# ziqin-h/GIVEPose

Measured on AMD Instinct MI355X. Metric: images/sec PoseNet fwd, bs=64 256x256 fp16, 1/2/4/8 MI355X; % MFMA roofline, higher is better.
Workload: dtype f16

## Files before the change

givepose_amd/_lib.py:

```python
import ctypes
import os
from ctypes import POINTER, Structure, c_char_p, c_double, c_float, c_int, c_long, c_void_p

_HERE = os.path.dirname(os.path.abspath(__file__))
LIB_PATH = os.environ.get("GP_LIB_PATH") or os.path.join(_HERE, "libgivepose_hip.so")

ABI_VERSION = 328
GP_F32, GP_F16, GP_F64 = 0, 1, 2
ACT_NONE, ACT_GELU, ACT_RELU, ACT_LRELU = 0, 1, 2, 3
EPI_NONE, EPI_GELU, EPI_RELU, EPI_LRELU, EPI_SCALE_RES, EPI_RES_RELU, EPI_LNFOLD_GELU = 0, 1, 2, 3, 4, 5, 6
ROT_6D, ROT_6D_Y, ROT_6D_Z, ROT_QUAT, ROT_EULER = 0, 1, 2, 3, 4
KC_GEMM, KC_DCNV3, KC_DWCONV_LN, KC_NORM, KC_ELEMENTWISE, KC_SMALL, KC_COUNT = 0, 1, 2, 3, 4, 5, 6
KC_NAMES = ["gemm", "dcnv3", "dwconv_ln", "norm", "elementwise", "small"]


class GemmDesc(Structure):
    _fields_ = [("X", c_void_p), ("W", c_void_p), ("bias", c_void_p), ("gamma", c_void_p), ("residual", c_void_p),
                ("C", c_void_p), ("workspace", c_void_p),
                ("M", c_int), ("N", c_int), ("K", c_int), ("ldx", c_int), ("ldc", c_int), ("ldres", c_int),
                ("epilogue", c_int), ("out_f32", c_int), ("splitk", c_int),
                ("B", c_int), ("H", c_int), ("Win", c_int), ("Cin", c_int), ("KH", c_int), ("KW", c_int),
                ("stride", c_int), ("pad", c_int), ("Ho", c_int), ("Wo", c_int), ("dtype", c_int),
                ("gn_partial", c_void_p), ("gn_groups", c_int), ("gn_hw", c_int), ("variant", c_int),
                ("ln_stats", c_void_p), ("ln_colsum", c_void_p), ("ln_nslab", c_int), ("ln_eps", c_float),
# ... 339 lines not shown
}
GPR_CHUNK, GPR_REPACK_LAUNCHES, GPR_REPACK_LAUNCHES_F32, GPR_MAX_ENTRIES, GPR_MAX_DIMS = 4096, 4, 3, 65536, 4
GPR_KIND_F32, GPR_KIND_F16, GPR_KIND_SPLIT = 0, 1, 2

TRAINDATA_PROTOTYPES = {
    "gpt_crop_train": ([_P] * 21 + [c_int] * 7 + [_P], c_int),
    "gpt_mask_deform": ([_P] * 3 + [c_ulonglong, _P, c_int, c_int, _P], c_int),
}
GPT_MAX_PIXELS, GPT_TRAIN_BATCH_LAUNCHES = 65536, 2

WPACK_PROTOTYPES = {
    "gpw_conv3_pack_wcm": ([_P, _P, c_int, c_int, _P], c_int),
    "gpw_gemm_desc_bytes": ([], c_int),
}

COLORAUG_PROTOTYPES = {
    "gpca_luma_partials": ([_P] * 5 + [c_int] * 3 + [_P], c_int),
    "gpca_apply": ([_P] * 6 + [c_int] * 3 + [_P], c_int),
}
GPCA_OP_SKIP, GPCA_OP_NONE, GPCA_OP_SHARPNESS, GPCA_OP_CONTRAST, GPCA_OP_BRIGHTNESS, GPCA_OP_COLOR = -1, 0, 1, 2, 3, 4
GPCA_BUF_FRAMES, GPCA_BUF_TMP0, GPCA_BUF_TMP1, GPCA_BUF_OUT = 0, 1, 2, 3
GPCA_PARTIALS, GPCA_STAGE_LAUNCHES, GPCA_MAX_FRAMES = 64, 2, 65535

_lib = None


class GivePoseHipError(RuntimeError):
    pass


# ... 2 lines not shown
    if _lib is not None:
        return _lib
    if not os.path.exists(LIB_PATH):
        raise GivePoseHipError(
            f"{LIB_PATH} not found: build it with `python -m givepose_amd.build` (hipcc --offload-arch=gfx950). "
            "There is no CPU or PyTorch fallback for the product path.")
    lib = ctypes.CDLL(LIB_PATH)
    for name, (argtypes, restype) in (list(PROTOTYPES.items()) + list(ALIGN_PROTOTYPES.items()) + list(LOSS_PROTOTYPES.items())
                                      + list(GRAD_PROTOTYPES.items()) + list(HEADGRAD_PROTOTYPES.items())
                                      + list(XYZGRAD_PROTOTYPES.items()) + list(XYZGRAD_BF16_PROTOTYPES.items()) + list(ENCGRAD_PROTOTYPES.items())
                                      + list(ENCGRAD_ORDERED_PROTOTYPES.items())
                                      + list(BBGRAD_PROTOTYPES.items()) + list(BBGRAD_BF16_PROTOTYPES.items()) + list(OPTIM_PROTOTYPES.items())
                                      + list(SIZEGRAD_PROTOTYPES.items()) + list(ACCUM_PROTOTYPES.items())
                                      + list(REPACK_PROTOTYPES.items()) + list(TRAINDATA_PROTOTYPES.items())
                                      + list(ADAM_PROTOTYPES.items()) + list(WPACK_PROTOTYPES.items())
                                      + list(COLORAUG_PROTOTYPES.items())):
        fn = getattr(lib, name)
        fn.argtypes = argtypes
        fn.restype = restype
    if lib.gp_version() != ABI_VERSION:
        raise GivePoseHipError(f"{LIB_PATH}: ABI version {lib.gp_version()}, this package needs {ABI_VERSION}: rebuild with "
                               "`python -m givepose_amd.build`")
    if lib.gpw_gemm_desc_bytes() != ctypes.sizeof(GemmDesc):
        raise GivePoseHipError(f"{LIB_PATH}: gp_gemm_desc is {lib.gpw_gemm_desc_bytes()} bytes there, {ctypes.sizeof(GemmDesc)} here: rebuild with "
                               "`python -m givepose_amd.build`")
    _lib = lib
    return lib


def check(rc, what=""):
    if rc != 0:
# ... 10 lines not shown
```

givepose_amd/build.py:

```python
import os
import subprocess
import sys

HERE = os.path.dirname(os.path.abspath(__file__))
CSRC = os.path.join(HERE, "csrc")
OBJ = os.path.join(HERE, "csrc", "build")
LIB = os.path.join(HERE, "libgivepose_hip.so")
SOURCES = ["runtime.hip", "gemm.hip", "mlp.hip", "dcnv3.hip", "dcnv3_any.hip", "norm.hip", "misc.hip", "scalenet.hip", "evalmap.hip", "align.hip", "loss.hip", "lossgrad.hip", "pnpgrad.hip", "xyzgrad.hip", "encgrad.hip", "encscatter.hip", "bbgrad.hip", "optim.hip", "sizegrad.hip", "accum.hip", "repack.hip", "traindata.hip", "adam.hip", "coloraug.hip"]
HIPCC = os.environ.get("HIPCC", "/opt/rocm/bin/hipcc")
FLAGS = ["-O3", "--offload-arch=gfx950", "-fPIC", "-std=c++17", "-Wno-unused-value"]
if os.environ.get("GP_PACKED_FP32") != "1":
    FLAGS += ["-Xclang", "-target-feature", "-Xclang", "-packed-fp32-ops", "-Wno-unknown-warning-option"]
EXTRA = os.environ.get("GP_EXTRA_HIPCC_FLAGS", "").split()
TAG = os.environ.get("GP_BUILD_TAG", "")
if EXTRA and not TAG:
    raise RuntimeError("GP_EXTRA_HIPCC_FLAGS needs GP_BUILD_TAG: an investigation build must not overwrite the product library")
if TAG:
    OBJ = os.path.join(HERE, "csrc", "build", "tag_" + TAG)
    LIB = os.path.join(HERE, f"libgivepose_hip_{TAG}.so")
    FLAGS += EXTRA


def _newer(a, b):
    return not os.path.exists(b) or os.path.getmtime(a) > os.path.getmtime(b)
# ... 1 lines not shown

def build(force=False, verbose=True):
    os.makedirs(OBJ, exist_ok=True)
    deps = [os.path.join(CSRC, "common.hpp"), os.path.join(HERE, "..", "include", "givepose_hip.h"),
            os.path.join(HERE, "..", "include", "givepose_align.h"), os.path.join(CSRC, "align_math.hpp"),
            os.path.join(HERE, "..", "include", "givepose_loss.h"), os.path.join(HERE, "..", "include", "givepose_grad.h"),
            os.path.join(HERE, "..", "include", "givepose_headgrad.h"), os.path.join(HERE, "..", "include", "givepose_xyzgrad.h"),
            os.path.join(HERE, "..", "include", "givepose_encgrad.h"), os.path.join(HERE, "..", "include", "givepose_bbgrad.h"),
            os.path.join(HERE, "..", "include", "givepose_optim.h"), os.path.join(HERE, "..", "include", "givepose_sizegrad.h"),
            os.path.join(HERE, "..", "include", "givepose_accum.h"), os.path.join(HERE, "..", "include", "givepose_repack.h"),
            os.path.join(HERE, "..", "include", "givepose_traindata.h"), os.path.join(CSRC, "grad_gemm.hpp"), os.path.join(CSRC, "grad_gemm_bf16.hpp"),
            os.path.join(HERE, "..", "include", "givepose_bbgrad_bf16.h"), os.path.join(CSRC, "xyz_conv_prec.hpp"),
            os.path.join(HERE, "..", "include", "givepose_xyzgrad_bf16.h"),
            os.path.join(HERE, "..", "include", "givepose_encgrad_ordered.h"), os.path.join(CSRC, "encscatter.hpp"),
            os.path.join(HERE, "..", "include", "givepose_adam.h"), os.path.join(HERE, "..", "include", "givepose_wpack.h"),
            os.path.join(HERE, "..", "include", "givepose_coloraug.h")]
    objs, procs = [], []
    for src in SOURCES:
        s, o = os.path.join(CSRC, src), os.path.join(OBJ, src.replace(".hip", ".o"))
        objs.append(o)
        if force or _newer(s, o) or any(_newer(d, o) for d in deps):
            if verbose:
                print("hipcc", src, flush=True)
            procs.append((src, subprocess.Popen([HIPCC, *FLAGS, "-c", s, "-o", o])))
    for src, p in procs:
        if p.wait() != 0:
            raise RuntimeError(f"hipcc failed on {src}")
    if force or procs or not os.path.exists(LIB) or any(_newer(o, LIB) for o in objs):
        subprocess.check_call([HIPCC, "--offload-arch=gfx950", "-shared", "-fPIC", "-o", LIB, *objs])
        if verbose:
            print("linked", LIB)
# ... 6 lines not shown
```

givepose_amd/csrc/mlp.hip:

```cpp
#include "common.hpp"

namespace {

struct MlpKP {
    const half_t* X;
    const half_t* W1;
    const float* b1;
    const half_t* W2p;
    const float* b2;
    const float* gamma;
    const half_t* res;
    half_t* out;
    int M;
    int dbg;
};

typedef __attribute__((address_space(3))) char lds_char_t;

__device__ __forceinline__ void glds16(const void* gsrc, unsigned lds_addr) {
    unsigned keep;
    asm volatile("s_mov_b32 %0, m0\n\ts_mov_b32 m0, %2\n\ts_nop 0\n\tglobal_load_lds_dwordx4 %1, off\n\ts_mov_b32 m0, %0"
                 : "=&s"(keep)
                 : "v"(gsrc), "s"(lds_addr)
                 : "memory");
}

__device__ __forceinline__ void glds16_sb(const void* sbase, unsigned voff, unsigned lds_addr) {
    unsigned keep;
    asm volatile("s_mov_b32 %0, m0\n\ts_mov_b32 m0, %3\n\ts_nop 0\n\tglobal_load_lds_dwordx4 %1, %2\n\ts_mov_b32 m0, %0"
// ... 8 lines not shown

#ifndef GP_MLP_WGS
#define GP_MLP_WGS 3
#endif
template <int C, int G16, int NWV = 8>
__global__ __launch_bounds__(NWV * 64, NWV == 4 ? GP_MLP_WGS : 1) void convnext_mlp_kernel(const MlpKP p) {
    constexpr int HD = 4 * C, NCH = HD / 32, KS = C / 32, CT = C / 16, MT = 2;
    constexpr int ROWB = C * 2;
    constexpr int W1B = 32 * ROWB, W2B = C * 64;
    constexpr int STAGE = W1B + W2B, NS = (NWV == 4 && C == 256) ? 2 : (NWV == 4 && GP_MLP_WGS == 3) ? 3 : 4, LEAD = NS - 1;
    constexpr int I1 = W1B / 1024 / NWV, I2 = W2B / 1024 / NWV, G = I1 + I2;
    constexpr int CPR1 = ROWB / 16, RPI1 = 64 / CPR1;
    constexpr int PITCH = ROWB + 16, SLAB = 32 * PITCH;
    constexpr int RING = NS * STAGE, SMEM = (RING + HD * 4) > NWV * SLAB ? (RING + HD * 4) : NWV * SLAB;
    static_assert(SMEM <= 160 * 1024, "LDS");
    __shared__ __attribute__((aligned(1024))) char smem[SMEM];

    const int tid = threadIdx.x, lane = tid & 63;
    const int wave = __builtin_amdgcn_readfirstlane(tid >> 6);
    const int fr = lane & 15, fq = lane >> 4;
    const long m0 = (long)xcd_chunk(blockIdx.x, gridDim.x) * (NWV * 32) + wave * 32;

    float* b1s = reinterpret_cast<float*>(smem + RING);
    for (int i = tid; i < HD / 4; i += NWV * 64) reinterpret_cast<f32x4*>(b1s)[i] = reinterpret_cast<const f32x4*>(p.b1)[i];

    uint4 xf[MT][KS];
#pragma unroll
    for (int mt = 0; mt < MT; ++mt)
#pragma unroll
        for (int ks = 0; ks < KS; ++ks)
            xf[mt][ks] = *reinterpret_cast<const uint4*>(p.X + (m0 + mt * 16 + fr) * C + ks * 32 + fq * 8);

    constexpr bool SB = true;
    unsigned w1off[I1], w2off[I2];
#pragma unroll
    for (int i = 0; i < I1; ++i) {
        const int r = (i * NWV + wave) * RPI1 + lane / CPR1, pc = lane % CPR1;
        w1off[i] = (unsigned)((r * C + ((pc ^ (r & 15)) << 3)) * 2);
    }
#pragma unroll
    for (int i = 0; i < I2; ++i) {
        const int lr = lane >> 2, r = (i * NWV + wave) * 16 + lr;
        w2off[i] = (unsigned)((r * HD + (((lane & 3) ^ ((-(lr >> 2)) & 3)) << 3)) * 2);
    }
    const unsigned lds0 = (unsigned)(size_t)(lds_char_t*)smem;
    auto stage = [&](int buf, int ch) {
        const unsigned s1 = lds0 + buf * STAGE + wave * 1024, s2 = s1 + W1B;
        const char* b1p = reinterpret_cast<const char*>(p.W1) + (long)ch * W1B;
        const char* b2p = reinterpret_cast<const char*>(p.W2p) + (long)ch * 64;
#pragma unroll
        for (int i = 0; i < I1; ++i) {
            if constexpr (SB) glds16_sb(b1p, w1off[i], s1 + i * NWV * 1024);
            else glds16(b1p + w1off[i], s1 + i * NWV * 1024);
        }
#pragma unroll
        for (int i = 0; i < I2; ++i) {
            if constexpr (SB) glds16_sb(b2p, w2off[i], s2 + i * NWV * 1024);
            else glds16(b2p + w2off[i], s2 + i * NWV * 1024);
        }
    };

    f32x4 acc2[CT][MT];
#pragma unroll
    for (int ct = 0; ct < CT; ++ct) {
        const f32x4 b = *reinterpret_cast<const f32x4*>(p.b2 + ct * 16 + fq * 4);
#pragma unroll
        for (int mt = 0; mt < MT; ++mt) acc2[ct][mt] = b;
    }
    __syncthreads();

#pragma unroll
    for (int i = 0; i < LEAD; ++i) stage(i, i);

    const int w1fo = fr * ROWB, w2fo = fr * 64 + ((fq ^ ((-(fr >> 2)) & 3)) << 4);
    int buf = 0, nbuf = LEAD;
    for (int ch = 0; ch < NCH; ++ch) {
        if (LEAD >= 3 && ch + 2 < NCH) asm volatile("s_waitcnt vmcnt(%0)" ::"n"(2 * G) : "memory");
        else if (LEAD >= 2 && ch + 1 < NCH) asm volatile("s_waitcnt vmcnt(%0)" ::"n"(G) : "memory");
        else asm volatile("s_waitcnt vmcnt(0)" ::: "memory");
        __builtin_amdgcn_s_barrier();
        __builtin_amdgcn_sched_barrier(0);
        if (ch + LEAD < NCH && p.dbg != 2) stage(nbuf, ch + LEAD);
        const char* s1 = smem + buf * STAGE + w1fo;
        const char* s2 = smem + buf * STAGE + W1B + w2fo;

        constexpr int GK = KS > 4 ? 1 : KS;
        f32x4 acc1[2][MT];
#pragma unroll
        for (int nt = 0; nt < 2; ++nt) {
            const f32x4 b = *reinterpret_cast<const f32x4*>(b1s + ch * 32 + nt * 16 + fq * 4);
#pragma unroll
            for (int mt = 0; mt < MT; ++mt) acc1[nt][mt] = b;
        }
#pragma unroll
        for (int k0 = 0; k0 < KS; k0 += GK) {
            uint4 a1[GK][2];
#pragma unroll
            for (int ks = 0; ks < GK; ++ks)
#pragma unroll
                for (int nt = 0; nt < 2; ++nt)
                    a1[ks][nt] = *reinterpret_cast<const uint4*>(s1 + nt * 16 * ROWB + ((((k0 + ks) * 4 + fq) ^ fr) << 4));
            __builtin_amdgcn_sched_barrier(0);
#pragma unroll
            for (int ks = 0; ks < GK; ++ks)
#pragma unroll
                for (int nt = 0; nt < 2; ++nt)
#pragma unroll
                    for (int mt = 0; mt < MT; ++mt) acc1[nt][mt] = mma16(a1[ks][nt], xf[mt][k0 + ks], acc1[nt][mt]);
            __builtin_amdgcn_sched_barrier(0);
        }
        constexpr int GC = CT > 8 ? 2 : (NWV == 4 && GP_MLP_WGS == 3) ? 4 : CT;
        uint4 a2[GC];
#pragma unroll
        for (int ct = 0; ct < GC; ++ct) a2[ct] = *reinterpret_cast<const uint4*>(s2 + ct * 1024);
        __builtin_amdgcn_sched_barrier(0);
        f32x2 v[8];
#pragma unroll
        for (int mt = 0; mt < MT; ++mt)
#pragma unroll
            for (int nt = 0; nt < 2; ++nt) {
                v[(mt * 2 + nt) * 2 + 0] = f32x2{acc1[nt][mt][0], acc1[nt][mt][1]};
                v[(mt * 2 + nt) * 2 + 1] = f32x2{acc1[nt][mt][2], acc1[nt][mt][3]};
            }
        uint4 hb[MT];
// ... 37 lines not shown
#pragma unroll
        for (int c0 = 0; c0 < CT; c0 += GC) {
            if (c0 > 0) {
#pragma unroll
                for (int ct = 0; ct < GC; ++ct) a2[ct] = *reinterpret_cast<const uint4*>(s2 + (c0 + ct) * 1024);
                __builtin_amdgcn_sched_barrier(0);
            }
#pragma unroll
            for (int ct = 0; ct < GC; ++ct)
#pragma unroll
                for (int mt = 0; mt < MT; ++mt) acc2[c0 + ct][mt] = mma16(a2[ct], hb[mt], acc2[c0 + ct][mt]);
            __builtin_amdgcn_sched_barrier(0);
        }
        buf = buf + 1 == NS ? 0 : buf + 1;
        nbuf = nbuf + 1 == NS ? 0 : nbuf + 1;
    }
    __syncthreads();

    constexpr int LPR = ROWB / 16, RPS = 64 / LPR, NIT = 32 / RPS;
    const int rr = lane / LPR, rc = lane % LPR;
    half8 rres[NIT];
    if constexpr (C == 128) {
#pragma unroll
        for (int i = 0; i < NIT; ++i) rres[i] = *reinterpret_cast<const half8*>(p.res + (m0 + i * RPS + rr) * C + rc * 8);
    }
    char* slab = smem + wave * SLAB;
#pragma unroll
    for (int ct = 0; ct < CT; ++ct) {
        const f32x4 g = *reinterpret_cast<const f32x4*>(p.gamma + ct * 16 + fq * 4);
#pragma unroll
// ... 415 lines not shown
    if (e != hipSuccess) return gp_fail(GP_ERR_LAUNCH, "gp_convnext_mlp_pack_w2_s32: %s", hipGetErrorString(e));
    return GP_OK;
}

extern "C" int gp_convnext_mlp_pack_w2(const void* w2, void* w2p, int C, void* stream) {
    GP_REQUIRE(w2 && w2p && w2 != w2p, "gp_convnext_mlp_pack_w2: bad pointers");
    GP_REQUIRE(C == 128 || C == 256 || C == 512, "gp_convnext_mlp_pack_w2: C=%d must be 128, 256 or 512", C);
    const long n = (long)C * 4 * C;
    hipLaunchKernelGGL(mlp_pack_w2_kernel, dim3(cdiv(n, 256)), dim3(256), 0, (hipStream_t)stream,
                       reinterpret_cast<const half_t*>(w2), reinterpret_cast<half_t*>(w2p), C, 4 * C);
    hipError_t e = hipGetLastError();
    if (e != hipSuccess) return gp_fail(GP_ERR_LAUNCH, "gp_convnext_mlp_pack_w2: %s", hipGetErrorString(e));
    return GP_OK;
}

extern "C" int gp_convnext_mlp(const void* x, const void* w1, const float* b1, const void* w2p, const float* b2,
                               const float* gamma, const void* residual, void* out, long M, int C, int dtype_in, void* stream) {
    const bool s32 = (dtype_in & GP_MLP_S32) != 0;
    const int dtype = dtype_in & ~GP_MLP_S32;
    GP_REQUIRE(dtype == GP_F16, "gp_convnext_mlp: fp16 storage only (fp32 runs fc1 / fc2 through gp_gemm)");
    GP_REQUIRE(!s32 || (C == 128 && gp_gelu16_enabled()), "gp_convnext_mlp: GP_MLP_S32 exists for C = 128 with the packed-fp16 GELU");
    GP_REQUIRE(C == 128 || C == 256 || C == 512, "gp_convnext_mlp: C=%d must be 128, 256 or 512", C);
    GP_REQUIRE(M > 0 && M % (C == 512 ? 128 : 256) == 0, "gp_convnext_mlp: M=%ld must be a positive multiple of %d", M, C == 512 ? 128 : 256);
    GP_REQUIRE(x && w1 && b1 && w2p && b2 && gamma && residual && out, "gp_convnext_mlp: null operand");
    GP_REQUIRE((((size_t)x | (size_t)w1 | (size_t)w2p | (size_t)residual | (size_t)out | (size_t)b1 | (size_t)b2 | (size_t)gamma) & 15) == 0,
               "gp_convnext_mlp: operands must be 16-byte aligned");
    GP_REQUIRE(x != out, "gp_convnext_mlp: x and out must not alias (out may alias residual)");
    MlpKP p;
    p.X = reinterpret_cast<const half_t*>(x); p.W1 = reinterpret_cast<const half_t*>(w1); p.b1 = b1;
    p.W2p = reinterpret_cast<const half_t*>(w2p); p.b2 = b2; p.gamma = gamma;
    p.res = reinterpret_cast<const half_t*>(residual); p.out = reinterpret_cast<half_t*>(out); p.M = (int)M;
    { const char* e = getenv("GP_MLP_DBG"); p.dbg = e ? atoi(e) : 0; }
    hipStream_t s = (hipStream_t)stream;
    const double flops = 2.0 * 2.0 * (double)M * C * 4 * C;
    const double bytes = 3.0 * M * C * 2 + 2.0 * 4 * C * C * 2;
    gp_timing_before(s, GP_KC_GEMM, flops, bytes);
    gp_timing_label("convnext_mlp C%d M%ld", C, M);
    if (C == 512) {
        const dim3 grid512((unsigned)(M / 128));
        GP_REQUIRE(gp_gelu16_enabled(), "gp_convnext_mlp: the C = 512 kernel exists with the packed-fp16 GELU only (GP_GELU16=0: run fc1 / fc2 through gp_gemm)");
        hipLaunchKernelGGL(convnext_mlp512_kernel, grid512, dim3(256), 0, s, p);
        GP_LAUNCH_CHECK("gp_convnext_mlp");
    }
    if (s32) {
        gp_timing_label("convnext_mlp s32 C%d M%ld", C, M);
        GP_REQUIRE(C == 128, "gp_convnext_mlp: GP_MLP_S32 is built for C = 128 (C = 256 needs 128 accumulator + 64 x registers beside a 16-register GEMM1 accumulator: it spilled 55)");
        hipLaunchKernelGGL((convnext_mlp_s32_kernel<128, 4>), dim3((unsigned)(M / 128)), dim3(256), 0, s, p);
        GP_LAUNCH_CHECK("gp_convnext_mlp");
    }
    const dim3 grid((unsigned)(M / 256));
    static const int mlp_waves = [] { const char* e = getenv("GP_MLP_WAVES"); return e ? atoi(e) : 4; }();
    if (gp_gelu16_enabled() && C == 128 && mlp_waves == 4) {
        hipLaunchKernelGGL((convnext_mlp_kernel<128, 1, 4>), dim3((unsigned)(M / 128)), dim3(256), 0, s, p);
        GP_LAUNCH_CHECK("gp_convnext_mlp");
    }
    if (gp_gelu16_enabled()) {
        if (C == 128) hipLaunchKernelGGL((convnext_mlp_kernel<128, 1>), grid, dim3(512), 0, s, p);
        else hipLaunchKernelGGL((convnext_mlp_kernel<256, 1>), grid, dim3(512), 0, s, p);
    } else {
        if (C == 128) hipLaunchKernelGGL((convnext_mlp_kernel<128, 0>), grid, dim3(512), 0, s, p);
        else hipLaunchKernelGGL((convnext_mlp_kernel<256, 0>), grid, dim3(512), 0, s, p);
    }
    GP_LAUNCH_CHECK("gp_convnext_mlp");
}
```

givepose_amd/ops.py:

```python
import ctypes
import os

import torch

from . import _lib
from ._lib import (ACT_GELU, ACT_LRELU, ACT_NONE, ACT_RELU, EPI_GELU, EPI_LNFOLD_GELU, EPI_LRELU, EPI_NONE, EPI_RELU, EPI_RES_RELU,
                   EPI_SCALE_RES, GP_F16, GP_F32, GP_F64, GemmDesc, check)

__all__ = ["dtype_code", "gemm", "conv2d_nhwc", "dcnv3_forward", "dcnv3_backward", "dcnv3_forward_into", "dcnv3_xyz_project", "convnext_stem", "dwconv_ln",
           "layernorm", "groupnorm", "upsample_bilinear2x", "deconv_col2im", "xyz_out_layer", "pointwise_k3",
           "pnp_conv1", "pnp_conv1_masked", "pool_mmm", "xyz_conv3x3_s2", "size_head", "pose_tail", "pose_tail_rt", "mask_resize_nearest"]


def _L():
    return _lib.load()


def _stream():
    return ctypes.c_void_p(torch.cuda.current_stream().cuda_stream)


def dtype_code(dt):
    if dt == torch.float16:
        return GP_F16
# ... 330 lines not shown


MLP_S32 = 0x400


def convnext_mlp_pack_w2(w2, s32=False):
    _contig(_chk(w2, "w2", torch.float16), "w2")
    if w2.dim() != 2 or w2.shape[1] != 4 * w2.shape[0]:
        raise RuntimeError(f"w2: expected shape (C, 4C), got {tuple(w2.shape)}")
    out = torch.empty_like(w2)
    fn = _L().gp_convnext_mlp_pack_w2_s32 if s32 else _L().gp_convnext_mlp_pack_w2
    check(fn(_ptr(w2), _ptr(out), w2.shape[0], _stream()), "gp_convnext_mlp_pack_w2")
    return out


def convnext_mlp(x, w1, b1, w2p, b2, gamma, residual, out, s32=False):
    _chk(x, "x", torch.float16)
    if x.dim() != 2:
        raise RuntimeError(f"x: expected shape (M, C), got {tuple(x.shape)}")
    M, C = x.shape
    for t, name, dt, shape in ((x, "x", torch.float16, (M, C)), (w1, "w1", torch.float16, (4 * C, C)), (b1, "b1", torch.float32, (4 * C,)),
                               (w2p, "w2p", torch.float16, (C, 4 * C)), (b2, "b2", torch.float32, (C,)), (gamma, "gamma", torch.float32, (C,)),
                               (residual, "residual", torch.float16, (M, C)), (out, "out", torch.float16, (M, C))):
        _chk(t, name, dt)
        if tuple(t.shape) != shape:
            raise RuntimeError(f"{name}: expected shape {shape}, got {tuple(t.shape)}")
        _contig(t, name)
    check(_L().gp_convnext_mlp(_ptr(x), _ptr(w1), _ptr(b1), _ptr(w2p), _ptr(b2), _ptr(gamma), _ptr(residual),
                               _ptr(out), M, C, GP_F16 | (MLP_S32 if s32 else 0), _stream()), "gp_convnext_mlp")
    return out


def dwconv_ln(x, wt, bias, ln_w, ln_b, out, KS, eps=1e-6, act=ACT_NONE, n_pixels=None, out_planes=False):
    B, H, W_, C = x.shape
    n = B * H * W_ if n_pixels is None else n_pixels
    if out_planes and n != B * H * W_:
        raise RuntimeError("dwconv_ln(out_planes): whole tensor only")
    check(_L().gp_dwconv_ln(_ptr(_contig(x, "x")), _ptr(wt), _ptr(bias), _ptr(ln_w), _ptr(ln_b), _ptr(out), B, H, W_, C, KS,
                            eps, act, n, _planes_code(x, out_planes, out), _stream()), "gp_dwconv_ln")
    return out


def dwconv_ln_groups(x, wt, bias, ln_w, ln_b, out, KS, crop_group_start, eps=1e-6, act=ACT_NONE):
    B, H, W_, C = x.shape
# ... 196 lines not shown
```

givepose_amd/posenet.py:

```python
import ctypes
import functools
import os
from collections import OrderedDict

import numpy as np
import torch
import torch.nn as nn

from . import _lib, ops, synth
from ._lib import (ACT_GELU, ACT_RELU, EPI_GELU, EPI_LNFOLD_GELU, EPI_LRELU, EPI_NONE, EPI_SCALE_RES)
from .config import FLAT_OPS, ROT_TYPES, PoseNetConfig, validate

CONV3_WCM_LAYERS = (6, 7, 9, 10)
OM_LD = 128


def enc0_xyz_pack(sd, prefix="nocs_encoder.features.0.", dtype=torch.float32):
    f64 = lambda k: sd[prefix + k].detach().to(device="cpu", dtype=torch.float64)
    cw, cb = f64("conv.weight").reshape(256, -1), f64("conv.bias")
    iw, ib = f64("dcnv3.input_proj.weight"), f64("dcnv3.input_proj.bias")
    ow, ob = f64("dcnv3.output_proj.weight"), f64("dcnv3.output_proj.bias")
    fold = torch.cat([iw @ cw, (iw @ cb + ib)[:, None]], 1)
    m = torch.cat([ow[:, 64 * g:64 * g + 64] @ fold[64 * g:64 * g + 64] for g in range(4)], 1)
    return m.to(dtype).contiguous(), ob.to(dtype).contiguous()
# ... 226 lines not shown
                p = f"stages_{s}.downsample."
                W[f"ds{s}.ln_w"], W[f"ds{s}.ln_b"] = f32(g(p + "0.weight")), f32(g(p + "0.bias"))
                W[f"ds{s}.w"] = gw(g(p + "1.weight").permute(0, 2, 3, 1).reshape(d, -1))
                W[f"ds{s}.b"] = f32(g(p + "1.bias"))
            for b in range(n):
                p, q = f"stages_{s}.blocks.{b}.", f"s{s}b{b}."
                W[q + "dw_w"] = lowp(g(p + "conv_dw.weight").reshape(d, 49).t())
                W[q + "dw_b"] = f32(g(p + "conv_dw.bias"))
                W[q + "ln_w"], W[q + "ln_b"] = f32(g(p + "norm.weight")), f32(g(p + "norm.bias"))
                W[q + "fc1_w"], W[q + "fc1_b"] = gw(g(p + "mlp.fc1.weight")), f32(g(p + "mlp.fc1.bias"))
                W[q + "fc2_w"], W[q + "fc2_b"] = gw(g(p + "mlp.fc2.weight")), f32(g(p + "mlp.fc2.bias"))
                W[q + "gamma"] = f32(g(p + "gamma"))
                fuse512 = d == 512 and (cfg.fuse_mlp512 or os.environ.get("GP_FUSE_MLP512") == "1")
                if T == torch.float16 and (d in (128, 256) or fuse512) and cfg.fuse_mlp:
                    W[q + "fc2_wp"] = ops.convnext_mlp_pack_w2(W[q + "fc2_w"])
                if T == torch.float16 and d == 512 and cfg.defer_ln:
                    w1, lw, lb = g(p + "mlp.fc1.weight"), g(p + "norm.weight"), g(p + "norm.bias")
                    wg = (w1 * lw[None, :]).to(T)
                    W[q + "fc1_wg"] = lowp(wg)
                    W[q + "fc1_cs"] = f32(wg.float().sum(1))
                    W[q + "fc1_cb"] = f32(w1 @ lb + g(p + "mlp.fc1.bias"))
        for head in ("xyz_nocs_head", "xyz_deform_head"):
            h = lambda k: sd[f"{head}.{k}"]
            W[head + ".deconv_w"] = gw(h("features.0.weight").permute(2, 3, 1, 0).reshape(9 * 256, -1))
            W[head + ".gn0_w"], W[head + ".gn0_b"] = f32(h("features.1.weight")), f32(h("features.1.bias"))
            for i in (3, 4, 6, 7, 9, 10):
                W[f"{head}.c{i}_w"] = gw(h(f"features.{i}.conv.weight").permute(0, 2, 3, 1).reshape(256, -1))
                if T == torch.float16 and i in CONV3_WCM_LAYERS:
                    W[f"{head}.c{i}_wcm"] = ops.conv3_pack_wcm(W[f"{head}.c{i}_w"])
                W[f"{head}.c{i}_gw"], W[f"{head}.c{i}_gb"] = f32(h(f"features.{i}.norm.weight")), f32(h(f"features.{i}.norm.bias"))
# ... 275 lines not shown
                                    out16=buf.get(f"x{s}h"))
            x2d = x.view(-1, d)
            xh = buf.get(f"x{s}h")
            xin = x if xh is None else xh
            for b in range(n):
                q = f"s{s}b{b}."
                if (q + "fc1_wg") in W and x2d.shape[0] % 256 == 0 and x.shape[1] % 4 == 0 and x.shape[2] % 16 == 0:
                    t = ops.dwconv7_raw_stats(x, W[q + "dw_w"], W[q + "dw_b"], buf[f"t{s}"], buf["ln_stats"])
                    ops.gemm(t.view(-1, d), W[q + "fc1_wg"], buf[f"h{s}"], bias=W[q + "fc1_cb"], epilogue=EPI_LNFOLD_GELU,
                             ln=(buf["ln_stats"], W[q + "fc1_cs"], d // 128, 1e-6))
                    ops.gemm(buf[f"h{s}"], W[q + "fc2_w"], x2d, bias=W[q + "fc2_b"], epilogue=EPI_SCALE_RES,
                             gamma=W[q + "gamma"], residual=x2d)
                    continue
                t = ops.dwconv_ln(xin, W[q + "dw_w"], W[q + "dw_b"], W[q + "ln_w"], W[q + "ln_b"], buf[f"t{s}"], 7, out_planes=self.split_gemm)
                if (q + "fc2_wp") in W and x2d.shape[0] % 256 == 0 and B >= cfg.fuse_mlp_min_batch and (d != 512 or x2d.shape[0] >= 32768):
                    ops.convnext_mlp(t.view(-1, d), W[q + "fc1_w"], W[q + "fc1_b"], W[q + "fc2_wp"], W[q + "fc2_b"],
                                     W[q + "gamma"], x2d, x2d)
                    continue
                pl = self.split_gemm
                ops.gemm(t.view(-1, d), W[q + "fc1_w"], buf[f"h{s}"], bias=W[q + "fc1_b"], epilogue=EPI_GELU, prefetch=W[q + "fc2_w"],
                         x_planes=pl, out_planes=pl)
                ops.gemm(buf[f"h{s}"], W[q + "fc2_w"], x2d, bias=W[q + "fc2_b"], epilogue=EPI_SCALE_RES,
                         gamma=W[q + "gamma"], residual=x2d, x_planes=pl, out16=None if xh is None else xh.view(-1, d),
                         prefetch=W.get(f"ds{s + 1}.w") if b == n - 1 else None)
        if cfg.main_backbone == "convnext":
            feat = x
        fc = dims[-1]
        feat2d = feat.view(B * 64, fc)
        ops.size_head(feat.view(B, 64, fc), W["size.w1"], W["size.b1"], W["size.w2"], W["size.b2"], buf["mean_size"], buf["size"], buf["size_scratch"])
        self._xyz_head(W, "xyz_nocs_head", feat2d, B, buf, buf["nocs_nchw"], buf["nocs_nhwc4"])
        self._seq_encoder(B, plan)
        cat2d = buf["feat_cat"].view(B * 64, 512)
# ... 661 lines not shown
```

givepose_amd/repack.py:

```python
import ctypes
import os
from collections import OrderedDict, namedtuple

import torch

from . import _lib, synth
from .ops import SPLIT_SHIFT, SplitW

OM_LD = 128
F32, F16, SPLIT = "f32", "f16", "split"
_KIND = {F32: _lib.GPR_KIND_F32, F16: _lib.GPR_KIND_F16, SPLIT: _lib.GPR_KIND_SPLIT}
FOLD = "@"

Entry = namedtuple("Entry", "src dims strides offset dst dst_off kind")
BnFold = namedtuple("BnFold", "w b bn_w bn_b mean var w_out b_out C K eps")
MatFold = namedtuple("MatFold", "A a_off a_rs B b_off b_rs b_f64 add out32 o32_off ld32 out64 o64_off ld64 M N K level")
MATRIX_FOLD_KEYS = tuple(f"enc{li}.{k}" for li in range(3) for k in ("fold_w", "fold_b")) + ("enc0.xyz_m",)


CONV3_WCM_LAYERS = (6, 7, 9, 10)


class Plan:
    def __init__(self):
# ... 138 lines not shown
            f32(f"ds{s}.b", g(p + "1.bias"))
        for b in range(n):
            p, q = f"stages_{s}.blocks.{b}.", f"s{s}b{b}."
            lowp(q + "dw_w", g(p + "conv_dw.weight").reshape(d, 49).t())
            f32(q + "dw_b", g(p + "conv_dw.bias"))
            f32(q + "ln_w", g(p + "norm.weight"))
            f32(q + "ln_b", g(p + "norm.bias"))
            gw(q + "fc1_w", g(p + "mlp.fc1.weight"))
            f32(q + "fc1_b", g(p + "mlp.fc1.bias"))
            gw(q + "fc2_w", g(p + "mlp.fc2.weight"))
            f32(q + "fc2_b", g(p + "mlp.fc2.bias"))
            f32(q + "gamma", g(p + "gamma"))
            fuse512 = d == 512 and (cfg.fuse_mlp512 or os.environ.get("GP_FUSE_MLP512") == "1")
            if fp16 and (d in (128, 256) or fuse512) and cfg.fuse_mlp:
                put(q + "fc2_wp", _View("backbone." + p + "mlp.fc2.weight", (d * 4 * d // 32, 4, 2, 4), (32, 4, 16, 1)).reshape(d, 4 * d), F16)
    for head in ("xyz_nocs_head", "xyz_deform_head"):
        h = lambda k: sd(f"{head}.{k}")
        gw(head + ".deconv_w", h("features.0.weight").permute(2, 3, 1, 0).reshape(9 * 256, -1))
        f32(head + ".gn0_w", h("features.1.weight"))
        f32(head + ".gn0_b", h("features.1.bias"))
        for i in (3, 4, 6, 7, 9, 10):
            gw(f"{head}.c{i}_w", h(f"features.{i}.conv.weight").permute(0, 2, 3, 1).reshape(256, -1))
            if fp16 and i in CONV3_WCM_LAYERS:
                cin = int(manifest[f"{head}.features.{i}.conv.weight"][1])
                put(f"{head}.c{i}_wcm", _View(f"{head}.features.{i}.conv.weight", (256, cin // 32, 9, 32), (cin * 9, 32 * 9, 1, 9)).reshape(256, -1), F16)
            f32(f"{head}.c{i}_gw", h(f"features.{i}.norm.weight"))
            f32(f"{head}.c{i}_gb", h(f"features.{i}.norm.bias"))
        f32(head + ".out_w", h("out_layer.weight").reshape(3, 256))
        f32(head + ".out_b", h("out_layer.bias"))
    C, K = manifest["size_head.conv1.weight"][:2]
# ... 194 lines not shown
```

include/givepose_hip.h:

```cpp
#ifndef GIVEPOSE_HIP_H
#define GIVEPOSE_HIP_H

#ifdef __cplusplus
extern "C" {
#endif

enum gp_status { GP_OK = 0, GP_ERR_INVALID = -1, GP_ERR_LAUNCH = -2, GP_ERR_RUNTIME = -3 };
enum gp_dtype { GP_F32 = 0, GP_F16 = 1, GP_F64 = 2  };
#define GP_OUT_PLANES 0x100
#define GP_IN_F32 0x200
#define GP_SPLIT_SHIFT 11
enum gp_act { GP_ACT_NONE = 0, GP_ACT_GELU = 1, GP_ACT_RELU = 2, GP_ACT_LRELU = 3  };
enum gp_epilogue {
    GP_EPI_NONE = 0,
    GP_EPI_GELU = 1,
    GP_EPI_RELU = 2,
    GP_EPI_LRELU = 3,
    GP_EPI_SCALE_RES = 4,
    GP_EPI_RES_RELU = 5,
    GP_EPI_LNFOLD_GELU = 6
};

const char* gp_last_error(void);
#define GP_ABI_VERSION 328
// ... 48 lines not shown
    int residual_f32;
    void* c16;
    int ldc16;
    int gn_rows;
    const void* W_cm;
} gp_gemm_desc;
int gp_gemm_gn_rows(int M, int N, int K, int hw);
int gp_gemm(const gp_gemm_desc* d, void* stream);

int gp_split_planes(const float* x, void* planes, long rows, int cols, long ldx, long plane_stride, int split_shift,
                    void* stream);

int gp_convnext_mlp_pack_w2(const void* w2, void* w2p, int C, void* stream);
int gp_convnext_mlp_pack_w2_s32(const void* w2, void* w2p, int C, void* stream);
#define GP_MLP_S32 0x400
int gp_convnext_mlp(const void* x, const void* w1, const float* b1, const void* w2p, const float* b2,
                    const float* gamma, const void* residual, void* out, long M, int C, int dtype, void* stream);

int gp_convnext_stem(const float* img, const float* w, const float* b, const float* ln_w, const float* ln_b,
                     void* out, int B, int H, int W, int C0, float eps, int dtype, void* stream);

int gp_dwconv_ln(const void* x, const void* wt, const float* bias, const float* ln_w, const float* ln_b,
                 void* y, int B, int H, int W, int C, int KS, float eps, int act, long n_pixels, int dtype,
                 void* stream);

int gp_dwconv_ln_groups(const void* x, const void* wt, const float* bias, const float* ln_w, const float* ln_b, void* y, int B,
                        int H, int W, int C, int KS, float eps, int act, const int* crop_group_start, int dtype, void* stream);

int gp_dwconv7_raw_stats(const void* x, const void* wt, const float* bias, void* y, float* stats, int B, int H, int W,
                         int C, int dtype, void* stream);
// ... 127 lines not shown
```

Baseline: 13230.

## Add chunk-major fc2 weight layout and staggered wave-group staging to fused MLP

Adds a chunk-major repack of the ConvNeXt MLP fc2 weight so each K-chunk's W2 slice is contiguous, letting the fused kernel stage one dense block per chunk instead of strided 64-byte pieces. Also adds a staggered schedule for C=256: the two wave groups take turns issuing the global-to-LDS prefetch, one before fc1 and one after, with an extra barrier, so loads overlap compute on the other half. Both are on by default through environment switches. The cost is an extra packed weight copy, more barriers and flag checks, and alignment limits on the new layout.

```diff
diff --git a/givepose_amd/_lib.py b/givepose_amd/_lib.py
--- a/givepose_amd/_lib.py
+++ b/givepose_amd/_lib.py
@@ -377,6 +377,10 @@
     "gpw_gemm_desc_bytes": ([], c_int),
 }
 
+MLP_PROTOTYPES = {
+    "gpm_convnext_mlp_pack_w2_cm": ([_P, _P, c_int, _P], c_int),
+}
+
 COLORAUG_PROTOTYPES = {
     "gpca_luma_partials": ([_P] * 5 + [c_int] * 3 + [_P], c_int),
     "gpca_apply": ([_P] * 6 + [c_int] * 3 + [_P], c_int),
@@ -409,7 +413,7 @@
                                       + list(SIZEGRAD_PROTOTYPES.items()) + list(ACCUM_PROTOTYPES.items())
                                       + list(REPACK_PROTOTYPES.items()) + list(TRAINDATA_PROTOTYPES.items())
                                       + list(ADAM_PROTOTYPES.items()) + list(WPACK_PROTOTYPES.items())
-                                      + list(COLORAUG_PROTOTYPES.items())):
+                                      + list(COLORAUG_PROTOTYPES.items()) + list(MLP_PROTOTYPES.items())):
         fn = getattr(lib, name)
         fn.argtypes = argtypes
         fn.restype = restype
diff --git a/givepose_amd/build.py b/givepose_amd/build.py
--- a/givepose_amd/build.py
+++ b/givepose_amd/build.py
@@ -6,7 +6,7 @@
 CSRC = os.path.join(HERE, "csrc")
 OBJ = os.path.join(HERE, "csrc", "build")
 LIB = os.path.join(HERE, "libgivepose_hip.so")
-SOURCES = ["runtime.hip", "gemm.hip", "mlp.hip", "dcnv3.hip", "dcnv3_any.hip", "norm.hip", "misc.hip", "scalenet.hip", "evalmap.hip", "align.hip", "loss.hip", "lossgrad.hip", "pnpgrad.hip", "xyzgrad.hip", "encgrad.hip", "encscatter.hip", "bbgrad.hip", "optim.hip", "sizegrad.hip", "accum.hip", "repack.hip", "traindata.hip", "adam.hip", "coloraug.hip"]
+SOURCES = ["runtime.hip", "gemm.hip", "mlp.hip", "mlp_w2cm.hip", "dcnv3.hip", "dcnv3_any.hip", "norm.hip", "misc.hip", "scalenet.hip", "evalmap.hip", "align.hip", "loss.hip", "lossgrad.hip", "pnpgrad.hip", "xyzgrad.hip", "encgrad.hip", "encscatter.hip", "bbgrad.hip", "optim.hip", "sizegrad.hip", "accum.hip", "repack.hip", "traindata.hip", "adam.hip", "coloraug.hip"]
 HIPCC = os.environ.get("HIPCC", "/opt/rocm/bin/hipcc")
 FLAGS = ["-O3", "--offload-arch=gfx950", "-fPIC", "-std=c++17", "-Wno-unused-value"]
 if os.environ.get("GP_PACKED_FP32") != "1":
@@ -39,7 +39,7 @@
             os.path.join(HERE, "..", "include", "givepose_xyzgrad_bf16.h"),
             os.path.join(HERE, "..", "include", "givepose_encgrad_ordered.h"), os.path.join(CSRC, "encscatter.hpp"),
             os.path.join(HERE, "..", "include", "givepose_adam.h"), os.path.join(HERE, "..", "include", "givepose_wpack.h"),
-            os.path.join(HERE, "..", "include", "givepose_coloraug.h")]
+            os.path.join(HERE, "..", "include", "givepose_coloraug.h"), os.path.join(HERE, "..", "include", "givepose_mlp.h")]
     objs, procs = [], []
     for src in SOURCES:
         s, o = os.path.join(CSRC, src), os.path.join(OBJ, src.replace(".hip", ".o"))
diff --git a/givepose_amd/csrc/mlp.hip b/givepose_amd/csrc/mlp.hip
--- a/givepose_amd/csrc/mlp.hip
+++ b/givepose_amd/csrc/mlp.hip
@@ -13,6 +13,8 @@
     half_t* out;
     int M;
     int dbg;
+    int cm;
+    int stg;
 };
 
 typedef __attribute__((address_space(3))) char lds_char_t;
@@ -51,10 +53,13 @@
     constexpr int PITCH = ROWB + 16, SLAB = 32 * PITCH;
     constexpr int RING = NS * STAGE, SMEM = (RING + HD * 4) > NWV * SLAB ? (RING + HD * 4) : NWV * SLAB;
     static_assert(SMEM <= 160 * 1024, "LDS");
+    constexpr bool CAN_STG = C == 256 && G16 && NWV == 8 && NS == 4;
     __shared__ __attribute__((aligned(1024))) char smem[SMEM];
 
     const int tid = threadIdx.x, lane = tid & 63;
     const int wave = __builtin_amdgcn_readfirstlane(tid >> 6);
+    const bool stg = CAN_STG && p.stg != 0;
+    const int grp = wave >> 2;
     const int fr = lane & 15, fq = lane >> 4;
     const long m0 = (long)xcd_chunk(blockIdx.x, gridDim.x) * (NWV * 32) + wave * 32;
 
@@ -78,13 +83,13 @@
 #pragma unroll
     for (int i = 0; i < I2; ++i) {
         const int lr = lane >> 2, r = (i * NWV + wave) * 16 + lr;
-        w2off[i] = (unsigned)((r * HD + (((lane & 3) ^ ((-(lr >> 2)) & 3)) << 3)) * 2);
+        w2off[i] = (unsigned)((r * (p.cm ? 32 : HD) + (((lane & 3) ^ ((-(lr >> 2)) & 3)) << 3)) * 2);
     }
     const unsigned lds0 = (unsigned)(size_t)(lds_char_t*)smem;
     auto stage = [&](int buf, int ch) {
         const unsigned s1 = lds0 + buf * STAGE + wave * 1024, s2 = s1 + W1B;
         const char* b1p = reinterpret_cast<const char*>(p.W1) + (long)ch * W1B;
-        const char* b2p = reinterpret_cast<const char*>(p.W2p) + (long)ch * 64;
+        const char* b2p = reinterpret_cast<const char*>(p.W2p) + (long)ch * (p.cm ? W2B : 64);
 #pragma unroll
         for (int i = 0; i < I1; ++i) {
             if constexpr (SB) glds16_sb(b1p, w1off[i], s1 + i * NWV * 1024);
@@ -111,13 +116,22 @@
 
     const int w1fo = fr * ROWB, w2fo = fr * 64 + ((fq ^ ((-(fr >> 2)) & 3)) << 4);
     int buf = 0, nbuf = LEAD;
+    if (stg) {
+        if (grp) {
+            asm volatile("s_waitcnt vmcnt(%0)" ::"n"(2 * G) : "memory");
+            __builtin_amdgcn_s_barrier();
+        }
+        __builtin_amdgcn_sched_barrier(0);
+    }
     for (int ch = 0; ch < NCH; ++ch) {
-        if (LEAD >= 3 && ch + 2 < NCH) asm volatile("s_waitcnt vmcnt(%0)" ::"n"(2 * G) : "memory");
-        else if (LEAD >= 2 && ch + 1 < NCH) asm volatile("s_waitcnt vmcnt(%0)" ::"n"(G) : "memory");
-        else asm volatile("s_waitcnt vmcnt(0)" ::: "memory");
+        if (!stg || !grp) {
+            if (LEAD >= 3 && ch + 2 < NCH) asm volatile("s_waitcnt vmcnt(%0)" ::"n"(2 * G) : "memory");
+            else if (LEAD >= 2 && ch + 1 < NCH) asm volatile("s_waitcnt vmcnt(%0)" ::"n"(G) : "memory");
+            else asm volatile("s_waitcnt vmcnt(0)" ::: "memory");
+        }
         __builtin_amdgcn_s_barrier();
         __builtin_amdgcn_sched_barrier(0);
-        if (ch + LEAD < NCH && p.dbg != 2) stage(nbuf, ch + LEAD);
+        if (ch + LEAD < NCH && p.dbg != 2 && (!stg || grp)) stage(nbuf, ch + LEAD);
         const char* s1 = smem + buf * STAGE + w1fo;
         const char* s2 = smem + buf * STAGE + W1B + w2fo;
 
@@ -145,6 +159,19 @@
 #pragma unroll
                     for (int mt = 0; mt < MT; ++mt) acc1[nt][mt] = mma16(a1[ks][nt], xf[mt][k0 + ks], acc1[nt][mt]);
             __builtin_amdgcn_sched_barrier(0);
+        }
+        if (stg) {
+            __builtin_amdgcn_sched_barrier(0);
+            if (grp) {
+                if (ch + 3 < NCH) asm volatile("s_waitcnt vmcnt(%0)" ::"n"(2 * G) : "memory");
+                else if (ch + 2 < NCH) asm volatile("s_waitcnt vmcnt(%0)" ::"n"(G) : "memory");
+                else asm volatile("s_waitcnt vmcnt(0)" ::: "memory");
+            }
+            asm volatile("" ::: "memory");
+            __builtin_amdgcn_s_barrier();
+            asm volatile("" ::: "memory");
+            __builtin_amdgcn_sched_barrier(0);
+            if (!grp && ch + LEAD < NCH && p.dbg != 2) stage(nbuf, ch + LEAD);
         }
         constexpr int GC = CT > 8 ? 2 : (NWV == 4 && GP_MLP_WGS == 3) ? 4 : CT;
         uint4 a2[GC];
@@ -212,6 +239,9 @@
         }
         buf = buf + 1 == NS ? 0 : buf + 1;
         nbuf = nbuf + 1 == NS ? 0 : nbuf + 1;
+    }
+    if (stg) {
+        if (!grp) __builtin_amdgcn_s_barrier();
     }
     __syncthreads();
 
@@ -657,11 +687,24 @@
     return GP_OK;
 }
 
+static int mlp_layout_flags_ok(int dtype_in, int C, const void* w2p) {
+    const bool cm = (dtype_in & GP_MLP_W2CM) != 0;
+    GP_REQUIRE(!cm || !(dtype_in & GP_MLP_S32), "gp_convnext_mlp: GP_MLP_W2CM with GP_MLP_S32: the 32x32x16 kernel reads gp_convnext_mlp_pack_w2_s32's layout only");
+    GP_REQUIRE(!cm || C != 512, "gp_convnext_mlp: GP_MLP_W2CM exists for C = 128 and 256 (the C = 512 kernel reads gp_convnext_mlp_pack_w2's layout)");
+    GP_REQUIRE(!cm || ((size_t)w2p & 127) == 0, "gp_convnext_mlp: a chunk-major w2p (GP_MLP_W2CM) must be 128-byte aligned");
+    GP_REQUIRE(!((dtype_in & GP_MLP_ONE_BARRIER) && (dtype_in & GP_MLP_STAGGERED)), "gp_convnext_mlp: GP_MLP_ONE_BARRIER and GP_MLP_STAGGERED exclude each other");
+    GP_REQUIRE(!(dtype_in & GP_MLP_STAGGERED) || (C == 256 && !(dtype_in & GP_MLP_S32) && gp_gelu16_enabled()),
+               "gp_convnext_mlp: GP_MLP_STAGGERED exists for C = 256 with the packed-fp16 GELU");
+    return GP_OK;
+}
+
 extern "C" int gp_convnext_mlp(const void* x, const void* w1, const float* b1, const void* w2p, const float* b2,
                                const float* gamma, const void* residual, void* out, long M, int C, int dtype_in, void* stream) {
     const bool s32 = (dtype_in & GP_MLP_S32) != 0;
-    const int dtype = dtype_in & ~GP_MLP_S32;
+    const bool cm = (dtype_in & GP_MLP_W2CM) != 0;
+    const int dtype = dtype_in & ~(GP_MLP_S32 | GP_MLP_W2CM | GP_MLP_ONE_BARRIER | GP_MLP_STAGGERED);
     GP_REQUIRE(dtype == GP_F16, "gp_convnext_mlp: fp16 storage only (fp32 runs fc1 / fc2 through gp_gemm)");
+    if (int rc = mlp_layout_flags_ok(dtype_in, C, w2p)) return rc;
     GP_REQUIRE(!s32 || (C == 128 && gp_gelu16_enabled()), "gp_convnext_mlp: GP_MLP_S32 exists for C = 128 with the packed-fp16 GELU");
     GP_REQUIRE(C == 128 || C == 256 || C == 512, "gp_convnext_mlp: C=%d must be 128, 256 or 512", C);
     GP_REQUIRE(M > 0 && M % (C == 512 ? 128 : 256) == 0, "gp_convnext_mlp: M=%ld must be a positive multiple of %d", M, C == 512 ? 128 : 256);
@@ -669,11 +712,15 @@
     GP_REQUIRE((((size_t)x | (size_t)w1 | (size_t)w2p | (size_t)residual | (size_t)out | (size_t)b1 | (size_t)b2 | (size_t)gamma) & 15) == 0,
                "gp_convnext_mlp: operands must be 16-byte aligned");
     GP_REQUIRE(x != out, "gp_convnext_mlp: x and out must not alias (out may alias residual)");
+    static const int mlp_stagger = [] { const char* e = getenv("GP_MLP_STAGGER"); return e ? atoi(e) : 1; }();
+    const bool can_stg = C == 256 && !s32 && gp_gelu16_enabled();
+    const bool stg = can_stg && !(dtype_in & GP_MLP_ONE_BARRIER) && (mlp_stagger != 0 || (dtype_in & GP_MLP_STAGGERED));
     MlpKP p;
     p.X = reinterpret_cast<const half_t*>(x); p.W1 = reinterpret_cast<const half_t*>(w1); p.b1 = b1;
     p.W2p = reinterpret_cast<const half_t*>(w2p); p.b2 = b2; p.gamma = gamma;
     p.res = reinterpret_cast<const half_t*>(residual); p.out = reinterpret_cast<half_t*>(out); p.M = (int)M;
     { const char* e = getenv("GP_MLP_DBG"); p.dbg = e ? atoi(e) : 0; }
+    p.cm = cm; p.stg = stg;
     hipStream_t s = (hipStream_t)stream;
     const double flops = 2.0 * 2.0 * (double)M * C * 4 * C;
     const double bytes = 3.0 * M * C * 2 + 2.0 * 4 * C * C * 2;
@@ -693,9 +740,10 @@
     }
     const dim3 grid((unsigned)(M / 256));
     static const int mlp_waves = [] { const char* e = getenv("GP_MLP_WAVES"); return e ? atoi(e) : 4; }();
+    const char* entry = cm ? (stg ? "gp_convnext_mlp/w2cm_stagger" : "gp_convnext_mlp/w2cm") : (stg ? "gp_convnext_mlp/stagger" : "gp_convnext_mlp");
     if (gp_gelu16_enabled() && C == 128 && mlp_waves == 4) {
         hipLaunchKernelGGL((convnext_mlp_kernel<128, 1, 4>), dim3((unsigned)(M / 128)), dim3(256), 0, s, p);
-        GP_LAUNCH_CHECK("gp_convnext_mlp");
+        GP_LAUNCH_CHECK(entry);
     }
     if (gp_gelu16_enabled()) {
         if (C == 128) hipLaunchKernelGGL((convnext_mlp_kernel<128, 1>), grid, dim3(512), 0, s, p);
@@ -704,5 +752,5 @@
         if (C == 128) hipLaunchKernelGGL((convnext_mlp_kernel<128, 0>), grid, dim3(512), 0, s, p);
         else hipLaunchKernelGGL((convnext_mlp_kernel<256, 0>), grid, dim3(512), 0, s, p);
     }
-    GP_LAUNCH_CHECK("gp_convnext_mlp");
-}
+    GP_LAUNCH_CHECK(entry);
+}
diff --git a/givepose_amd/csrc/mlp_w2cm.hip b/givepose_amd/csrc/mlp_w2cm.hip
--- /dev/null
+++ b/givepose_amd/csrc/mlp_w2cm.hip
@@ -0,0 +1,25 @@
+#include "common.hpp"
+#include "../../include/givepose_mlp.h"
+
+namespace {
+
+__global__ void mlp_pack_w2_cm_kernel(const half_t* w2, half_t* w2cm, int C, int HD) {
+    const long i = (long)blockIdx.x * 256 + threadIdx.x;
+    if (i >= (long)C * HD) return;
+    const int t = (int)(i & 31), c = (int)((i >> 5) % C), ch = (int)((i >> 5) / C);
+    const int fq = t >> 3, nt = (t >> 2) & 1, j = t & 3;
+    w2cm[i] = w2[(long)c * HD + ch * 32 + nt * 16 + fq * 4 + j];
+}
+
+}
+
+extern "C" int gpm_convnext_mlp_pack_w2_cm(const void* w2, void* w2cm, int C, void* stream) {
+    GP_REQUIRE(w2 && w2cm && w2 != w2cm, "gpm_convnext_mlp_pack_w2_cm: bad pointers");
+    GP_REQUIRE(C == 128 || C == 256, "gpm_convnext_mlp_pack_w2_cm: C=%d must be 128 or 256", C);
+    const long n = (long)C * 4 * C;
+    hipLaunchKernelGGL(mlp_pack_w2_cm_kernel, dim3(cdiv(n, 256)), dim3(256), 0, (hipStream_t)stream,
+                       reinterpret_cast<const half_t*>(w2), reinterpret_cast<half_t*>(w2cm), C, 4 * C);
+    hipError_t e = hipGetLastError();
+    if (e != hipSuccess) return gp_fail(GP_ERR_LAUNCH, "gpm_convnext_mlp_pack_w2_cm: %s", hipGetErrorString(e));
+    return GP_OK;
+}
diff --git a/givepose_amd/ops.py b/givepose_amd/ops.py
--- a/givepose_amd/ops.py
+++ b/givepose_amd/ops.py
@@ -368,7 +368,28 @@
     return out
 
 
-def convnext_mlp(x, w1, b1, w2p, b2, gamma, residual, out, s32=False):
+MLP_W2CM = 0x800
+
+
+def mlp_w2cm():
+    return os.environ.get("GP_MLP_W2CM", "1")[:1] != "0"
+
+MLP_SCHEDULES = {None: 0, "one_barrier": 0x1000, "staggered": 0x2000}
+
+
+def convnext_mlp_pack_w2_cm(w2, out=None):
+    _contig(_chk(w2, "w2", torch.float16), "w2")
+    if w2.dim() != 2 or w2.shape[1] != 4 * w2.shape[0]:
+        raise RuntimeError(f"w2: expected shape (C, 4C), got {tuple(w2.shape)}")
+    if out is None:
+        out = torch.empty_like(w2)
+    elif out.dtype != torch.float16 or tuple(out.shape) != tuple(w2.shape) or not out.is_contiguous() or out.device != w2.device:
+        raise RuntimeError(f"out: expected a contiguous float16 {tuple(w2.shape)} tensor beside w2")
+    check(_L().gpm_convnext_mlp_pack_w2_cm(_ptr(w2), _ptr(out), w2.shape[0], _stream()), "gpm_convnext_mlp_pack_w2_cm")
+    return out
+
+
+def convnext_mlp(x, w1, b1, w2p, b2, gamma, residual, out, s32=False, w2cm=False, schedule=None):
     _chk(x, "x", torch.float16)
     if x.dim() != 2:
         raise RuntimeError(f"x: expected shape (M, C), got {tuple(x.shape)}")
@@ -381,7 +402,8 @@
             raise RuntimeError(f"{name}: expected shape {shape}, got {tuple(t.shape)}")
         _contig(t, name)
     check(_L().gp_convnext_mlp(_ptr(x), _ptr(w1), _ptr(b1), _ptr(w2p), _ptr(b2), _ptr(gamma), _ptr(residual),
-                               _ptr(out), M, C, GP_F16 | (MLP_S32 if s32 else 0), _stream()), "gp_convnext_mlp")
+                               _ptr(out), M, C, GP_F16 | (MLP_S32 if s32 else 0) | (MLP_W2CM if w2cm else 0) | MLP_SCHEDULES[schedule], _stream()),
+          "gp_convnext_mlp")
     return out
 
 
diff --git a/givepose_amd/posenet.py b/givepose_amd/posenet.py
--- a/givepose_amd/posenet.py
+++ b/givepose_amd/posenet.py
@@ -264,6 +264,8 @@
                 fuse512 = d == 512 and (cfg.fuse_mlp512 or os.environ.get("GP_FUSE_MLP512") == "1")
                 if T == torch.float16 and (d in (128, 256) or fuse512) and cfg.fuse_mlp:
                     W[q + "fc2_wp"] = ops.convnext_mlp_pack_w2(W[q + "fc2_w"])
+                    if d in (128, 256) and ops.mlp_w2cm():
+                        W[q + "fc2_w2cm"] = ops.convnext_mlp_pack_w2_cm(W[q + "fc2_w"])
                 if T == torch.float16 and d == 512 and cfg.defer_ln:
                     w1, lw, lb = g(p + "mlp.fc1.weight"), g(p + "norm.weight"), g(p + "norm.bias")
                     wg = (w1 * lw[None, :]).to(T)
@@ -569,8 +571,9 @@
                     continue
                 t = ops.dwconv_ln(xin, W[q + "dw_w"], W[q + "dw_b"], W[q + "ln_w"], W[q + "ln_b"], buf[f"t{s}"], 7, out_planes=self.split_gemm)
                 if (q + "fc2_wp") in W and x2d.shape[0] % 256 == 0 and B >= cfg.fuse_mlp_min_batch and (d != 512 or x2d.shape[0] >= 32768):
-                    ops.convnext_mlp(t.view(-1, d), W[q + "fc1_w"], W[q + "fc1_b"], W[q + "fc2_wp"], W[q + "fc2_b"],
-                                     W[q + "gamma"], x2d, x2d)
+                    wcm = W.get(q + "fc2_w2cm")
+                    ops.convnext_mlp(t.view(-1, d), W[q + "fc1_w"], W[q + "fc1_b"], W[q + "fc2_wp"] if wcm is None else wcm, W[q + "fc2_b"],
+                                     W[q + "gamma"], x2d, x2d, w2cm=wcm is not None)
                     continue
                 pl = self.split_gemm
                 ops.gemm(t.view(-1, d), W[q + "fc1_w"], buf[f"h{s}"], bias=W[q + "fc1_b"], epilogue=EPI_GELU, prefetch=W[q + "fc2_w"],
diff --git a/givepose_amd/repack.py b/givepose_amd/repack.py
--- a/givepose_amd/repack.py
+++ b/givepose_amd/repack.py
@@ -5,7 +5,7 @@
 import torch
 
 from . import _lib, synth
-from .ops import SPLIT_SHIFT, SplitW
+from .ops import SPLIT_SHIFT, SplitW, mlp_w2cm
 
 OM_LD = 128
 F32, F16, SPLIT = "f32", "f16", "split"
@@ -176,6 +176,10 @@
             fuse512 = d == 512 and (cfg.fuse_mlp512 or os.environ.get("GP_FUSE_MLP512") == "1")
             if fp16 and (d in (128, 256) or fuse512) and cfg.fuse_mlp:
                 put(q + "fc2_wp", _View("backbone." + p + "mlp.fc2.weight", (d * 4 * d // 32, 4, 2, 4), (32, 4, 16, 1)).reshape(d, 4 * d), F16)
+                if d in (128, 256) and mlp_w2cm():
+                    for ch in range(4 * d // 32):
+                        put(q + "fc2_w2cm", _View("backbone." + p + "mlp.fc2.weight", (d, 4, 2, 4), (4 * d, 4, 16, 1), offset=ch * 32), F16,
+                            dst_off=ch * d * 32, shape=(d, 4 * d))
     for head in ("xyz_nocs_head", "xyz_deform_head"):
         h = lambda k: sd(f"{head}.{k}")
         gw(head + ".deconv_w", h("features.0.weight").permute(2, 3, 1, 0).reshape(9 * 256, -1))
diff --git a/include/givepose_hip.h b/include/givepose_hip.h
--- a/include/givepose_hip.h
+++ b/include/givepose_hip.h
@@ -86,6 +86,9 @@
 int gp_convnext_mlp_pack_w2(const void* w2, void* w2p, int C, void* stream);
 int gp_convnext_mlp_pack_w2_s32(const void* w2, void* w2p, int C, void* stream);
 #define GP_MLP_S32 0x400
+#define GP_MLP_W2CM 0x800
+#define GP_MLP_ONE_BARRIER 0x1000
+#define GP_MLP_STAGGERED 0x2000
 int gp_convnext_mlp(const void* x, const void* w1, const float* b1, const void* w2p, const float* b2,
                     const float* gamma, const void* residual, void* out, long M, int C, int dtype, void* stream);
 
diff --git a/include/givepose_mlp.h b/include/givepose_mlp.h
--- /dev/null
+++ b/include/givepose_mlp.h
@@ -0,0 +1,15 @@
+#ifndef GIVEPOSE_MLP_H
+#define GIVEPOSE_MLP_H
+
+#include "givepose_hip.h"
+
+#ifdef __cplusplus
+extern "C" {
+#endif
+
+int gpm_convnext_mlp_pack_w2_cm(const void* w2, void* w2cm, int C, void* stream);
+
+#ifdef __cplusplus
+}
+#endif
+#endif
```

Result: no change. 13190 (-0.3%).
